# CAMMA-public/SelfPose3d

Measured on AMD Instinct MI355X. Metric: multi-view samples/sec (5-view Panoptic, 80x80x20 voxel), higher is better.
Workload: dtype f32

## Files before the change

include/sp3d.h:

```cpp
#ifndef SP3D_H
#define SP3D_H

#include <stdint.h>

#ifdef __cplusplus
extern "C" {
#endif

#define SP3D_ABI_VERSION 3
#define SP3D_MAX_VIEWS 16
#define SP3D_MAX_TOPK 32

#define SP3D_CAM_STRIDE 64
#define SP3D_CAM_R 0
#define SP3D_CAM_T 9
#define SP3D_CAM_F 12
#define SP3D_CAM_C 14
#define SP3D_CAM_K 16
#define SP3D_CAM_P 19
#define SP3D_CAM_A 21
#define SP3D_CAM_W0 27
#define SP3D_CAM_H0 28
#define SP3D_CAM_FLIP 29
#define SP3D_CAM_RXY 32
// ... 143 lines not shown
                          int64_t sPk, int64_t sQj, int64_t sQk, int conj_p, int conj_q, void *stream);

int sp3d_wino_input(const float *x, float *V, int B, int X, int Y, int Z, int C, void *stream);
int sp3d_wino_output(const float *M, float *y, const float *shift, const float *residual, int mode, int B, int X, int Y,
                     int Z, int O, void *stream);
int sp3d_wino_fused(const float *x, const float *U, float *y, const float *shift, const float *residual, int mode, int B,
                    int X, int Y, int Z, int C, int O, void *stream);

int sp3d_wino_fused_split(const float *x, const void *U3, float *y, const float *shift, const float *residual, int mode, int B,
                          int X, int Y, int Z, int C, int O, void *stream);

int sp3d_wino_fused_split64(const float *x, const void *U3, float *y, const float *shift, const float *residual, int mode,
                            int B, int X, int Y, int Z, int C, int O, void *stream);

int sp3d_conv3_split(const float *x, const void *W3, float *y, const float *shift, const float *residual, int mode, int B,
                     int X, int Y, int Z, int C, int O, void *stream);

int sp3d_upsample2x_scatter(const float *G, float *out, const float *shift, const float *skip, int64_t batch, int X, int Y,
                            int Z, int O, void *stream);

int sp3d_upsample2x_scatter_head(const float *G, float *head, const float *shift, const float *skip, const float *wout,
                                 const float *bout, int64_t batch, int X, int Y, int Z, int O, int J, void *stream);

#define SP3D_GBN_F32 0
#define SP3D_GBN_F64 1
#define SP3D_GBN_REPLICAS 16
#define SP3D_GBN_PLAIN 0
#define SP3D_GBN_RELU 1
#define SP3D_GBN_ADD_RELU 2
int64_t sp3d_gbn_workspace_bytes(int G, int C);
int sp3d_gbn_forward(const void *x, void *y, int dtype, const int32_t *group_of, const int32_t *group_samples, int N,
                     int64_t S, int C, int G, int G_update, const void *weight, const void *bias, void *running_mean,
                     void *running_var, double eps, double momentum, int mode, const void *residual, void *mean,
                     void *invstd, void *scale, void *shift, double *workspace, void *stream);
int sp3d_gbn_backward(const void *x, const void *dy, void *dx, int dtype, const int32_t *group_of,
                      const int32_t *group_samples, int N, int64_t S, int C, int G, const void *weight, const void *mean,
                      const void *invstd, const void *scale, const void *shift, int mode, const void *y,
                      void *grad_residual, void *grad_weight, void *grad_bias, void *k123, double *workspace, void *stream);

#ifdef __cplusplus
}
#endif
#endif
```

selfpose3d_amd/_lib.py:

```python
from __future__ import annotations

import ctypes as C
import os
from typing import Optional, Sequence

import torch

_HERE = os.path.dirname(os.path.abspath(__file__))
_DEFAULT_LIB_PATH = os.path.join(_HERE, "libsp3d.so")
NOPK_LIB_PATH = os.path.join(_HERE, "libsp3d_nopk.so")
LIB_PATH = os.environ.get("SP3D_LIB_PATH") or _DEFAULT_LIB_PATH

LAYOUT_PLANAR = 0
LAYOUT_NHWC = 1
OUT_CHANNELS_LAST = 0x100
HM_BF16 = 0x200
OUT_BF16 = 0x400
HM_ONE_CHANNEL = 0x800
SCATTER_AUTO, SCATTER_PER_TAP, SCATTER_MERGE = 0, 2, 3
MAX_VIEWS = 16
MAX_TOPK = 32
ABI_VERSION = 3

_CTYPES = {"p": C.c_void_p, "i": C.c_int, "l": C.c_int64, "f": C.c_float, "d": C.c_double, "s": C.c_char_p}
# ... 42 lines not shown
    "sp3d_wino_input": "i: pp iiiii p",
    "sp3d_wino_output": "i: pppp iiiiii p",
    "sp3d_wino_fused": "i: ppppp iiiiiii p",
    "sp3d_wino_fused_split": "i: ppppp iiiiiii p",
    "sp3d_wino_fused_split64": "i: ppppp iiiiiii p",
    "sp3d_conv3_split": "i: ppppp iiiiiii p",
    "sp3d_upsample2x_scatter": "i: pppp l iiii p",
    "sp3d_upsample2x_scatter_head": "i: pppppp l iiiii p",
    "sp3d_gbn_workspace_bytes": "l: ii",
    "sp3d_gbn_forward": "i: pp i pp i l iii pppp dd i ppppppp",
    "sp3d_gbn_backward": "i: ppp i pp i l ii ppppp i ppppppp",
}
TUNING_SIGNATURES = {
    "sp3d_unproject_fwd_variant": "i: p i ppppp iiiiiiii p iii p",
    "sp3d_unproject_fwd_plan": "i: iii p iiiiiiiii pppp",
    "sp3d_debug_set_timeline": "i: p",
    "sp3d_debug_stamp": "i: pp",
}
ONE_TRAIN_SIGNATURES = {
    "sp3d_unproject_one_fwd_train": "i: p ii ppppppp iiiiiiii p ii p",
    "sp3d_unproject_one_bwd": "i: ppppp l pp iiiiiiii p ii p",
    "sp3d_unproject_one_bwd_det": "i: ppppp l ppp iiiiiiii p ii p",
}
EXPORTS = list(SIGNATURES)

_lib = None


class Sp3dError(RuntimeError):
    pass


def shared_gpu() -> bool:
    v = os.environ.get("SP3D_SHARED_GPU")
    if v is not None:
        return v.lower() in ("1", "true", "yes", "on")
    if any(os.environ.get(k) not in (None, "") for k in ("HIP_VISIBLE_DEVICES", "CUDA_VISIBLE_DEVICES", "ROCR_VISIBLE_DEVICES",
                                                          "GPU_DEVICE_ORDINAL")):
        return False
    try:
        ranks = int(os.environ.get("LOCAL_WORLD_SIZE", "1"))
        if ranks > 1 and torch.cuda.is_available() and ranks > torch.cuda.device_count():
            import warnings
            warnings.warn(f"selfpose3d_amd: {ranks} local ranks on {torch.cuda.device_count()} GPU(s) - ranks share a GPU: loading "
                          "libsp3d_nopk.so (no packed-fp32 instructions; set SP3D_SHARED_GPU=0 to force the default flavour)")
            return True
    except ValueError:
        pass
    return False


def load():
    global _lib, LIB_PATH
    if _lib is not None:
        return _lib
    if shared_gpu() and LIB_PATH == _DEFAULT_LIB_PATH:
        LIB_PATH = NOPK_LIB_PATH
    if not os.path.exists(LIB_PATH):
        raise Sp3dError(
            f"{LIB_PATH} not found - the HIP extension is not built. Run `python -m selfpose3d_amd.build` "
            "(hipcc, gfx950). There is no CPU fallback for the unprojection path.")
    lib = C.CDLL(LIB_PATH)
    for table, required in ((SIGNATURES, True), (ONE_TRAIN_SIGNATURES, True), (TUNING_SIGNATURES, False)):
        for name, sig in table.items():
            if required or hasattr(lib, name):
                ret, args = sig.split(":")
                fn = getattr(lib, name)
                fn.restype = _CTYPES[ret]
                fn.argtypes = [_CTYPES[a] for a in args.replace(" ", "")]
    if lib.sp3d_abi_version() != ABI_VERSION:
        raise Sp3dError(f"libsp3d.so ABI {lib.sp3d_abi_version()} != binding ABI {ABI_VERSION}; rebuild")
    _lib = lib
    return lib


def check(rc: int, what: str):
    if rc != 0:
        msg = load().sp3d_error_string(rc).decode()
        raise Sp3dError(f"{what} failed: {msg} (code {rc})")


def _stream(device) -> int:
    return torch.cuda.current_stream(device).cuda_stream


def _require_cuda(t: torch.Tensor, name: str):
# ... 645 lines not shown
                               _stream(x.device)), "sp3d_wino_output")
    return y


def wino_fused_conv3d_(x: torch.Tensor, U: torch.Tensor, shift: torch.Tensor, mode: int,
                       residual: Optional[torch.Tensor] = None, U3: Optional[torch.Tensor] = None) -> torch.Tensor:
    lib = load()
    _require_cuda(x, "x")
    B, Cc, X, Y, Z = (int(v) for v in x.shape)
    _require_cl3d_f32(x, "wino_fused_conv3d_")
    O = int(U.shape[2])
    y = _empty_cl3d(B, O, X, Y, Z, x.device)
    if residual is not None:
        residual = _as_cl3d(residual)
    if U3 is None:
        name, weights = "sp3d_wino_fused", U
    else:
        name, weights = ("sp3d_wino_fused_split64" if O == 64 else "sp3d_wino_fused_split"), U3
    check(getattr(lib, name)(x.data_ptr(), weights.data_ptr(), y.data_ptr(), shift.data_ptr(), _opt(residual), int(mode),
                             B, X, Y, Z, Cc, O, _stream(x.device)), name)
    return y


def upsample2x_(x: torch.Tensor, w_gemm: torch.Tensor, shift: torch.Tensor, skip: torch.Tensor) -> torch.Tensor:
    lib = load()
    _require_cuda(x, "x")
    B, Cc, X, Y, Z = (int(v) for v in x.shape)
    _require_cl3d_f32(x, "upsample2x_")
    O = int(w_gemm.shape[1]) // 8
    G = torch.matmul(x.permute(0, 2, 3, 4, 1).reshape(-1, Cc), w_gemm)
    out = _empty_cl3d(B, O, 2 * X, 2 * Y, 2 * Z, x.device)
    skip = _as_cl3d(skip)
    check(lib.sp3d_upsample2x_scatter(G.data_ptr(), out.data_ptr(), shift.data_ptr(), skip.data_ptr(), B, X, Y, Z, O,
                                      _stream(x.device)), "sp3d_upsample2x_scatter")
    return out


def upsample2x_head_(x: torch.Tensor, w_gemm: torch.Tensor, shift: torch.Tensor, skip: torch.Tensor, w_out: torch.Tensor,
                     b_out: torch.Tensor) -> torch.Tensor:
    lib = load()
    _require_cuda(x, "x")
    B, Cc, X, Y, Z = (int(v) for v in x.shape)
    _require_cl3d_f32(x, "upsample2x_head_")
    O = int(w_gemm.shape[1]) // 8
    J = int(w_out.shape[0])
    G = torch.matmul(x.permute(0, 2, 3, 4, 1).reshape(-1, Cc), w_gemm)
    skip = _as_cl3d(skip)
    wo = w_out.reshape(J, O).contiguous().float()
    bo = (b_out if b_out is not None else torch.zeros(J, device=x.device)).contiguous().float()
    head = _empty_cl3d(B, J, 2 * X, 2 * Y, 2 * Z, x.device)
    check(lib.sp3d_upsample2x_scatter_head(G.data_ptr(), head.data_ptr(), shift.data_ptr(), skip.data_ptr(), wo.data_ptr(),
                                           bo.data_ptr(), B, X, Y, Z, O, J, _stream(x.device)), "sp3d_upsample2x_scatter_head")
    return head


class _RenderJoints(torch.autograd.Function):
    @staticmethod
    def forward(ctx, kps, count, h, w, sigma):
        lib = load()
        _require_cuda(kps, "kps")
        N, Pn, J = (int(v) for v in kps.shape[:3])
        k = kps.contiguous().float()
        cnt = None if count is None else count.to(device=kps.device, dtype=torch.int32).contiguous()
        out = torch.empty((N, J, h, w), dtype=torch.float32, device=kps.device)
        check(lib.sp3d_render_joints_fwd(k.data_ptr(), _opt(cnt), N, Pn, J, h, w, float(sigma), out.data_ptr(),
                                         _stream(kps.device)), "sp3d_render_joints_fwd")
        ctx.save_for_backward(k, cnt if cnt is not None else torch.empty(0, device=kps.device))
        ctx.geom = (h, w, float(sigma), cnt is not None, kps.dtype)
        return out if kps.dtype == torch.float32 else out.to(kps.dtype)

    @staticmethod
    def backward(ctx, gout):
        lib = load()
# ... 13 lines not shown
```

selfpose3d_amd/build.py:

```python
from __future__ import annotations

import os
import subprocess
import sys

HERE = os.path.dirname(os.path.abspath(__file__))
CSRC = os.path.join(HERE, "csrc")
SOURCES = ["sp3d_unproject.hip", "sp3d_proposal.hip", "sp3d_epilogue.hip", "sp3d_synth.hip", "sp3d_fftconv.hip", "sp3d_winograd.hip", "sp3d_fft.hip", "sp3d_gbn.hip"]
HEADERS = [os.path.join("..", "pk_src1.py"), "sp3d_device.h", "sp3d_proj_pk.h", "sp3d_tuning.h", "sp3d_twiddles.h", os.path.join("..", "..", "include", "sp3d.h"),
           os.path.join("..", "..", "include", "sp3d_one_train.h")]
LIB = os.path.join(HERE, "libsp3d.so")
HIPCC = os.environ.get("HIPCC", "/opt/rocm/bin/hipcc")
FLAGS = ["--offload-arch=gfx950", "-O3", "-std=c++17", "-ffp-contract=off", "-munsafe-fp-atomics", "-fPIC", "-shared",
         "-Wall", "-Wno-unused-function"]
LINK = ["-L/opt/rocm/lib", "-lhipfft"]


def needs_build() -> bool:
    if not os.path.exists(LIB):
        return True
    t = os.path.getmtime(LIB)
    deps = [os.path.join(CSRC, s) for s in SOURCES + HEADERS] + [os.path.abspath(__file__)]
    return any(os.path.getmtime(d) > t for d in deps if os.path.exists(d))


PER_SOURCE_FLAGS = {"sp3d_winograd.hip": ["-fno-slp-vectorize"],
                    "sp3d_fft.hip": ["-fno-slp-vectorize"], "sp3d_fftconv.hip": ["-fno-slp-vectorize"]}


LLVM_BIN = os.environ.get("SP3D_LLVM_BIN", "/opt/rocm/lib/llvm/bin")

NOPK_LIB = os.path.join(HERE, "libsp3d_nopk.so")
NOPK_FLAGS = ["-DSP3D_NO_PK", "-fno-slp-vectorize", "-Xclang", "-target-feature", "-Xclang", "-packed-fp32-ops"]




def _compile_one(src: str, objdir: str, cflags, verbose: bool, host_flags=()) -> str:
    from . import pk_src1
    base = os.path.join(objdir, src.replace(".hip", ""))
    path = os.path.join(CSRC, src)
    cuid = "-cuid=" + src.replace(".", "_")

    def run(cmd):
        if verbose:
            print(" ".join(cmd))
        subprocess.check_call(cmd)
    if os.environ.get("SP3D_PLAIN_HIPCC", "0") not in ("", "0"):
        flags = cflags + [f for f in NOPK_FLAGS if f not in cflags]
# ... 78 lines not shown
```

selfpose3d_amd/csrc/sp3d_winograd.hip:

```cpp
#include <hip/hip_runtime.h>
#include <stdint.h>

#include "../../include/sp3d.h"

namespace sp3d {

__device__ __forceinline__ void bt4(float &d0, float &d1, float &d2, float &d3)
{
    const float t0 = d0 - d2, t1 = d1 + d2, t2 = d2 - d1, t3 = d1 - d3;
    d0 = t0; d1 = t1; d2 = t2; d3 = t3;
}

__global__ __launch_bounds__(256) void wino_input_kernel(const float *__restrict__ x, float *__restrict__ V, int B, int X,
                                                        int Y, int Z, int C, int TX, int TY, int TZ)
{
    const int64_t T = (int64_t)B * TX * TY * TZ;
    const int64_t gid = (int64_t)blockIdx.x * 256 + threadIdx.x;
    if (gid >= T * C) return;
    const int c = (int)(gid % C);
    int64_t t = gid / C;
    const int tz = (int)(t % TZ); int64_t r = t / TZ;
    const int ty = (int)(r % TY); r /= TY;
    const int tx = (int)(r % TX);
    const int b = (int)(r / TX);
    float d[4][4][4];
#pragma unroll
// ... 119 lines not shown
extern "C" int sp3d_wino_output(const float *M, float *y, const float *shift, const float *residual, int mode, int B, int X,
                                int Y, int Z, int O, void *stream)
{
    if (B <= 0 || X <= 0 || Y <= 0 || Z <= 0 || O <= 0 || mode < 0 || mode > 3) return SP3D_EINVAL;
    if (!M || !y || !shift || (mode >= 2 && !residual)) return SP3D_ENULL;
    const int TX = (X + 1) / 2, TY = (Y + 1) / 2, TZ = (Z + 1) / 2;
    const int64_t n = (int64_t)B * TX * TY * TZ * O;
    if ((n + 255) / 256 > 0x7fffffff) return SP3D_ERANGE;
    const dim3 grid((unsigned)((n + 255) / 256)), block(256);
    hipStream_t s = (hipStream_t)stream;
#define SP3D_WO(MODE_) hipLaunchKernelGGL((wino_output_kernel<MODE_>), grid, block, 0, s, M, y, shift, residual, B, X, Y, Z, O, TX, TY, TZ)
    switch (mode) { case 0: SP3D_WO(0); break; case 1: SP3D_WO(1); break; case 2: SP3D_WO(2); break; default: SP3D_WO(3); }
#undef SP3D_WO
    const hipError_t e = hipGetLastError();
    return e == hipSuccess ? SP3D_OK : (int)e;
}

#ifndef SP3D_W16_ABLATE
#define SP3D_W16_ABLATE 0
#endif

namespace sp3d {

typedef float f32x16 __attribute__((ext_vector_type(16)));
#ifdef SP3D_WF_TIMELINE
__device__ unsigned long long *g_wf_tl = nullptr;
#define WF_STAMP(slot) do { __builtin_amdgcn_sched_barrier(0); if (tl && lane == 0) tl[slot] = __builtin_readcyclecounter(); __builtin_amdgcn_sched_barrier(0); } while (0)
#else
#define WF_STAMP(slot) do { } while (0)
#endif

constexpr int WF_RX = 10, WF_RY = 10, WF_RZ = 6;
constexpr int WF_VS = 8;
constexpr int WF_ROW = WF_RX * WF_VS + 4;
constexpr int WF_LDS = WF_RY * WF_RZ * WF_ROW;

__device__ constexpr int wf_ta(int r) { return r == 0 ? 0 : (r == 1 ? 1 : (r == 2 ? 2 : 1)); }
__device__ constexpr int wf_tb(int r) { return r == 0 ? 2 : (r == 1 ? 2 : (r == 2 ? 1 : 3)); }
__device__ constexpr float wf_sb(int r) { return r == 1 ? 1.0f : -1.0f; }
__device__ constexpr float wf_at(int a, int r) { return a == 0 ? (r < 3 ? 1.0f : 0.0f) : (r == 0 ? 0.0f : (r == 1 ? 1.0f : -1.0f)); }

template <int C, int MODE>
__global__ __launch_bounds__(64) void wino_fused_kernel(const float *__restrict__ x, const float *__restrict__ U,
                                                       float *__restrict__ y, const float *__restrict__ shift,
                                                       const float *__restrict__ res, int B, int X, int Y, int Z, int NBX,
                                                       int NBY, int NBZ)
{
// ... 130 lines not shown
                const int rx = row & 3, ry = (row >> 2) & 3, rz = row >> 4;
                const int xo = min(ox0 + 2 * rx + (a >> 2), X - 1), yo = min(oy0 + 2 * ry + ((a >> 1) & 1), Y - 1);
                const int zo = min(oz0 + 2 * rz + (a & 1), Z - 1);
                rv[v] = res[((((int64_t)b * X + xo) * Y + yo) * Z + zo) * O + t];
            }
        }
#pragma unroll
        for (int v = 0; v < 16; ++v) {
            const int row = 8 * (v >> 2) + (v & 3) + 4 * h;
            const int rx = row & 3, ry = (row >> 2) & 3, rz = row >> 4;
            const int xo = ox0 + 2 * rx + (a >> 2), yo = oy0 + 2 * ry + ((a >> 1) & 1), zo = oz0 + 2 * rz + (a & 1);
            if (xo < X && yo < Y && zo < Z) {
                const int64_t idx = ((((int64_t)b * X + xo) * Y + yo) * Z + zo) * O + t;
                float val = acc[a][v] + sh;
                if (MODE == 2) val += rv[v];
                if (MODE >= 1) val = fmaxf(val, 0.0f);
                if (MODE == 3) val += rv[v];
                y[idx] = val;
            }
        }
    }
}


typedef unsigned u32x4 __attribute__((ext_vector_type(4)));
typedef unsigned u32x2 __attribute__((ext_vector_type(2)));
typedef unsigned u32x4_a8 __attribute__((ext_vector_type(4), aligned(8)));
typedef unsigned u32x2_a8 __attribute__((ext_vector_type(2), aligned(8)));
typedef __bf16 bf16x8 __attribute__((ext_vector_type(8)));
typedef __bf16 bf16x2 __attribute__((ext_vector_type(2)));
typedef float f32x2 __attribute__((ext_vector_type(2)));

__device__ __forceinline__ unsigned pack_bf16(float a, float b)
{
    f32x2 f = {a, b};
    return __builtin_bit_cast(unsigned, __builtin_convertvector(f, bf16x2));
}
__device__ __forceinline__ float bf16_lo(unsigned u) { return __uint_as_float(u << 16); }
__device__ __forceinline__ float bf16_hi(unsigned u) { return __uint_as_float(u & 0xffff0000u); }
__device__ __forceinline__ f32x16 mfma_bf16(u32x4 a, u32x4 b, f32x16 c)
{
    return __builtin_amdgcn_mfma_f32_32x32x16_bf16(__builtin_bit_cast(bf16x8, a), __builtin_bit_cast(bf16x8, b), c, 0, 0, 0);
}

struct WfB { u32x4 mh; u32x2 l; };

template <int C, int MODE>
__global__ __launch_bounds__(64) __attribute__((amdgpu_waves_per_eu(2, 2))) void wino_fused3_kernel(const float *__restrict__ x, const unsigned *__restrict__ U3,
                                                        float *__restrict__ y, const float *__restrict__ shift,
                                                        const float *__restrict__ res, int B, int X, int Y, int Z, int NBX,
                                                        int NBY, int NBZ)
{
    constexpr int O = 32, NCH = C / 8;
    __shared__ __attribute__((aligned(16))) float region[WF_LDS];
    const int lane = threadIdx.x, t = lane & 31, h = lane >> 5;
    int bid = blockIdx.x;
    const int bz = bid % NBZ; bid /= NBZ;
    const int by = bid % NBY; bid /= NBY;
    const int bx = bid % NBX;
    const int b = bid / NBX;
    const int ttx = t & 3, tty = (t >> 2) & 3, ttz = t >> 4;
    const int ox0 = bx * 8, oy0 = by * 8, oz0 = bz * 4;
    const float *rb = region + ((2 * ttz) * WF_RY + 2 * tty) * WF_ROW + (2 * ttx) * WF_VS + 4 * h;

    f32x16 acc[8];
#pragma unroll
// ... 471 lines not shown
constexpr int CD_BX = 16, CD_BY = 8, CD_BZ = 4;
constexpr int CD_RX = CD_BX + 2, CD_RY = CD_BY + 2, CD_RZ = CD_BZ + 2, CD_VOX = 8, CD_ROW = CD_RX * CD_VOX, CD_ZP = CD_RY * CD_ROW + 4;
constexpr int CD_PLANE = CD_RZ * CD_ZP;
constexpr int CD_BUF = 2 * CD_PLANE;
constexpr int CD_NV4 = CD_RX * CD_RY * CD_RZ * 2;
constexpr int CD_PROD = 4;
constexpr int CD_PER = (CD_NV4 + 64 * CD_PROD - 1) / (64 * CD_PROD);
constexpr int CD_BUFS = ((CD_BUF / 4 + 63) / 64) * 256;
#ifndef SP3D_WG_ABLATE
#define SP3D_WG_ABLATE 0
#endif
struct CdRec { u32x4 hl, hh, mm; };


#ifdef SP3D_CD_TIMELINE
__device__ unsigned long long *g_cd_tl = nullptr;
#define CD_STAMP(slot) do { __builtin_amdgcn_sched_barrier(0); if (g_cd_tl && blockIdx.x == 0 && lane == 0 && item < 64) { g_cd_tl[(wave * 64 + item) * 4 + (slot)] = __builtin_readcyclecounter(); \
     \
    if (wave == 0 && (slot) == 0 && item == 0) { g_cd_tl[(7 * 64 + 62) * 4 + 0] = wall_clock64(); g_cd_tl[(7 * 64 + 62) * 4 + 1] = __builtin_readcyclecounter(); } \
    if (wave == 0 && (slot) == 3) { g_cd_tl[(7 * 64 + 63) * 4 + 0] = wall_clock64(); g_cd_tl[(7 * 64 + 63) * 4 + 1] = __builtin_readcyclecounter(); } } __builtin_amdgcn_sched_barrier(0); } while (0)
#else
#define CD_STAMP(slot) do { (void)item; } while (0)
#endif

__device__ __forceinline__ void split3(const float4 a, u32x4 &q0, u32x4 &q1)
{
    const unsigned hi01 = pack_bf16(a.x, a.y), hi23 = pack_bf16(a.z, a.w);
    const float r0 = __builtin_amdgcn_fmed3f(a.x - bf16_lo(hi01), 0.0f, a.x - bf16_lo(hi01));
    const float r1 = __builtin_amdgcn_fmed3f(a.y - bf16_hi(hi01), 0.0f, a.y - bf16_hi(hi01));
    const float r2 = __builtin_amdgcn_fmed3f(a.z - bf16_lo(hi23), 0.0f, a.z - bf16_lo(hi23));
    const float r3 = __builtin_amdgcn_fmed3f(a.w - bf16_hi(hi23), 0.0f, a.w - bf16_hi(hi23));
    const unsigned mid01 = pack_bf16(r0, r1), mid23 = pack_bf16(r2, r3);
    const unsigned lo01 = pack_bf16(r0 - bf16_lo(mid01), r1 - bf16_hi(mid01));
    const unsigned lo23 = pack_bf16(r2 - bf16_lo(mid23), r3 - bf16_hi(mid23));
    q0 = u32x4{lo01, lo23, hi01, hi23};
    q1 = u32x4{hi01, hi23, mid01, mid23};
}

template <int C, int MODE>
__global__ __launch_bounds__(64 * (4 + CD_PROD)) __attribute__((amdgpu_waves_per_eu(2, 2)))
void conv3_split_kernel(const float *__restrict__ x, const unsigned *__restrict__ W3, float *__restrict__ y,
                        const float *__restrict__ shift, const float *__restrict__ res, int B, int X, int Y, int Z, int NBX,
                        int NBY, int NBZ, int nblocks)
{
    constexpr int O = 32, NCH = C / 8;
    extern __shared__ __attribute__((aligned(16))) unsigned cd_lds[];
    const int tid = threadIdx.x, lane = tid & 63, wave = tid >> 6, t = lane & 31, h = lane >> 5;
    const int my_blocks = ((int)blockIdx.x < nblocks) ? (nblocks - 1 - (int)blockIdx.x) / (int)gridDim.x + 1 : 0;
    const int n_items = my_blocks * NCH;
    auto decode = [&](int item, int &b, int &ox0, int &oy0, int &oz0) {
        int bid = (int)blockIdx.x + (item / NCH) * (int)gridDim.x;
        const int bz = bid % NBZ; bid /= NBZ;
        const int by = bid % NBY; bid /= NBY;
        const int bx = bid % NBX;
        b = bid / NBX;
        ox0 = bx * CD_BX; oy0 = by * CD_BY; oz0 = bz * CD_BZ;
    };

    if (wave >= 4) {
        const int pt = tid - 256;
// ... 322 lines not shown
```

selfpose3d_amd/v2v_net.py:

```python
from __future__ import annotations

from typing import NamedTuple, Optional

import torch
import torch.nn as nn
import torch.nn.functional as F


def _bn(c):
    from .grouped_bn import GroupedBatchNorm3d
    return GroupedBatchNorm3d(c)


def _grouped(bn, training: bool) -> bool:
    return training and getattr(bn, "groups", None) is not None


def fft_len(n: int) -> int:
    m = n + (n & 1)
    while True:
        r, odd = m, 0
        for q in (2, 3, 5, 7, 11, 13):
            if q > 2 and r % q == 0:
                odd += 1
# ... 179 lines not shown
        self.spec, self.X, self.Y, self.Z, self.SZ = spec, int(X), int(Y), int(Z), int(SZ)
        self.shape = (int(spec.shape[0]), int(spec.shape[1]), self.X, self.Y, self.Z)
        self.device, self.is_cuda, self.dtype = spec.device, spec.is_cuda, torch.float32


class _Conv(NamedTuple):
    w: torch.Tensor
    shift: torch.Tensor
    u: Optional[torch.Tensor] = None
    split: Optional[torch.Tensor] = None
    direct: Optional[torch.Tensor] = None


class _Res(NamedTuple):
    c1: _Conv
    c2: _Conv
    skip: Optional[torch.Tensor]


class _Up(NamedTuple):
    wT: torch.Tensor
    shift: torch.Tensor
    wg: torch.Tensor


class _FoldedV2V:

    def __init__(self, net: "V2VNet"):
        self.net = net
        self.key = None
        self.layers = {}
        self.spectra = {}
        self.xpad = {}

    def graph_tensors(self):
        return dict(self.layers), dict(self.spectra), dict(self.xpad)

    @staticmethod
    def _key(net):
        ps = list(net.parameters()) + list(net.buffers())
        w3 = net.front_layers[1].res_branch[0].weight
        return (tuple((p.data_ptr(), p._version) for p in ps), str(w3.device), bool(is_cl(w3)))

    def _ensure_built(self):
        key = self._key(self.net)
        if key != self.key:
# ... 2 lines not shown

    @staticmethod
    def _fold(conv, bn, transposed=False):
        s = bn.weight / torch.sqrt(bn.running_var + bn.eps)
        shape = (1, -1, 1, 1, 1) if transposed else (-1, 1, 1, 1, 1)
        w = conv.weight * s.view(shape)
        fmt = torch.channels_last_3d if is_cl(conv.weight) else torch.contiguous_format
        b = conv.bias if conv.bias is not None else torch.zeros_like(bn.running_mean)
        return w.contiguous(memory_format=fmt), ((b - bn.running_mean) * s + bn.bias).contiguous()

    @staticmethod
    def _conv3_record(w, shift):
        from . import _lib
        cout, cin = int(w.shape[0]), int(w.shape[1])
        routes = {conv3_route(cin, cout, (b, 2, 2, 2), True, ws, dc) for b in (1, 1 << 20) for ws in (True, False) for dc in (True, False)}
        if not w.is_cuda or routes == {"library"}:
            return _Conv(w, shift)
        u = _lib.wino_weights(w)
        split = _lib.wino_weights_split(u, 16 if cout == 64 else 8) if "wino_fused_conv3d_" in routes else None
        direct = _lib.conv_weights_split(w) if "conv3_split_" in routes else None
        return _Conv(w, shift, u, split, direct)

    def _build(self):
        n, layers = self.net, {}
        layers["front"] = _Conv(*self._fold(n.front_layers[0].block[0], n.front_layers[0].block[1]))
        ed = n.encoder_decoder
        for name in ("front_res", "encoder_res1", "encoder_res2", "mid_res", "decoder_res2", "decoder_res1", "skip_res1",
                     "skip_res2"):
            blk = n.front_layers[1] if name == "front_res" else getattr(ed, name)
            w1, s1 = self._fold(blk.res_branch[0], blk.res_branch[1])
            w2, s2 = self._fold(blk.res_branch[3], blk.res_branch[4])
            ws = None
            if len(blk.skip_con) > 0:
                ws, ss = self._fold(blk.skip_con[0], blk.skip_con[1])
                s2 = (s2 + ss).contiguous()
            layers[name] = _Res(self._conv3_record(w1, s1), self._conv3_record(w2, s2), ws)
        for name in ("decoder_upsample2", "decoder_upsample1"):
            blk = getattr(ed, name).block
            wT, sT = self._fold(blk[0], blk[1], transposed=True)
            wg = wT.permute(0, 2, 3, 4, 1).reshape(wT.shape[0], 8 * wT.shape[1]).contiguous()
            layers[name] = _Up(wT, sT, wg)
        self.layers, self.spectra, self.xpad = layers, {}, {}

    def _conv3(self, x, c: "_Conv", mode, residual=None):
        from . import _lib
        n, route = self.net, "library"
        split = getattr(n, "wino_split", True)
        if c.u is not None and is_cl(x):
            route = conv3_route(int(c.w.shape[1]), int(c.w.shape[0]), (x.shape[0],) + tuple(x.shape[2:]), n.winograd, split,
                                getattr(n, "direct_conv", True))
        if route == "conv3_split_":
            return _lib.conv3_split_(x, c.direct, c.shift, mode, residual)
        if route == "wino_fused_conv3d_":
            return _lib.wino_fused_conv3d_(x, c.u, c.shift, mode, residual, c.split if split else None)
        if route == "wino_conv3d_":
            return _lib.wino_conv3d_(x, c.u, c.shift, mode, residual)
        return _lib.channel_shift_act_(F.conv3d(x, c.w, None, 1, 1), c.shift, mode, residual)

    def _res(self, x, name):
        r = self.layers[name]
        h = self._conv3(x, r.c1, 1)
        return self._conv3(h, r.c2, 2, x if r.skip is None else self._conv1(x, r.skip))

    _tuned_shapes: "set[tuple]" = set()
# ... 153 lines not shown
        else:
            buf = self._fft_buffer(B, cin, S, x.device)
            buf[:, :, :X, :Y, :Z].copy_(x[:, :cin])
        Yf = _lib.freq_contract(_lib.rfft3d(buf), self._weights_f(w0, S))
        y = _lib.irfft3d_(Yf, S[2])
        cl = is_cl(self.layers["front_res"].c1.w)
        if cl and y.is_contiguous() and y.shape[1] % 4 == 0 and Z % 4 == 0 and 4 * Z * (y.shape[1] + 4) * 4 <= 65536:
            return _lib.crop_shift_act_cl(y, X, Y, Z, s0, True)
        y = y[:, :, :X, :Y, :Z]
        y = y.contiguous(memory_format=torch.channels_last_3d if cl else torch.contiguous_format)
        return _lib.channel_shift_act_(y, s0, 1)

    def _tail(self, x):
        from . import _lib
        x = self._res(x, "front_res")
        skip1 = self._res(x, "skip_res1")
        x = self._res(self._pool(x), "encoder_res1")
        skip2 = self._res(x, "skip_res2")
        x = self._res(self._pool(x), "encoder_res2")
        x = self._res(self._res(x, "mid_res"), "decoder_res2")
        x = self._up2x(x, "decoder_upsample2", skip2)
        x = self._res(x, "decoder_res1")
        o = self.net.output_layer
        wT, sT, wg = self.layers["decoder_upsample1"]
        if self.net.winograd and is_cl(x) and wg.is_cuda and wT.shape[1] == 32 and x.dtype == torch.float32:
            return _lib.upsample2x_head_(x, wg, sT, skip1, o.weight, o.bias)
        x = self._up2x(x, "decoder_upsample1", skip1)
        return self._conv1(x, o.weight, o.bias)

    def _pool(self, x):
        from . import _lib
        if is_cl(x) and x.is_cuda and x.dtype == torch.float32 and x.shape[1] % 4 == 0 and \
                all(int(v) % 2 == 0 for v in x.shape[2:]):
            return _lib.maxpool2x(x)
        return F.max_pool3d(x, 2, 2)

    def _up2x(self, x, name, skip):
        from . import _lib
        wT, sT, wg = self.layers[name]
        if self.net.winograd and is_cl(x) and wg.is_cuda and wT.shape[1] % 4 == 0:
            return _lib.upsample2x_(x, wg, sT, skip)
        return _lib.channel_shift_act_(F.conv_transpose3d(x, wT, None, 2), sT, 3, skip)

    def _conv1(self, x, w, bias=None):
        if self.net.winograd and is_cl(x) and x.is_cuda:
            B, C, X, Y, Z = x.shape
            O = w.shape[0]
            x2 = x.permute(0, 2, 3, 4, 1).reshape(-1, C)
            y = torch.matmul(x2, w.reshape(O, C).t()) if bias is None else torch.addmm(bias, x2, w.reshape(O, C).t())
            return y.view(B, X, Y, Z, O).permute(0, 4, 1, 2, 3)
        return F.conv3d(x, w, bias, 1, 0)


class V2VNet(nn.Module):
    def __init__(self, input_channels: int, output_channels: int):
        super().__init__()
        self.front_layers = nn.Sequential(ConvBnRelu3d(input_channels, 16, 7), Residual3d(16, 32))
        self.encoder_decoder = _EncDec()
        self.output_layer = nn.Conv3d(32, output_channels, 1, 1, 0)
        self.fused_inference = True
        self.fft_front = True
        self.winograd = True
        self.zdft = True
        self.wino_split = True
# ... 83 lines not shown
```

Measured before the change: 2767.

## Fuse transposed-conv GEMM with scatter epilogue and head into one MFMA kernel

Adds a HIP kernel that computes the 2x transposed-conv upsample directly with split-bf16 MFMA (three-piece fp32 emulation), then applies shift, ReLU and skip-add and writes the scattered output in one pass. For the final decoder layer it also applies the 1x1 output head in-kernel through an LDS transpose. This removes the intermediate GEMM result G and its separate scatter kernel, saving a round-trip through global memory. The cost is a more complex kernel restricted to two channel configurations, plus extra MFMA work from the 3-way split.

After: 2825 (median of 6 runs). +2.1%, better.

```diff
diff --git a/include/sp3d.h b/include/sp3d.h
--- a/include/sp3d.h
+++ b/include/sp3d.h
@@ -189,6 +189,8 @@
 int sp3d_upsample2x_scatter_head(const float *G, float *head, const float *shift, const float *skip, const float *wout,
                                  const float *bout, int64_t batch, int X, int Y, int Z, int O, int J, void *stream);
 
+#include "sp3d_upconv.h"
+
 #define SP3D_GBN_F32 0
 #define SP3D_GBN_F64 1
 #define SP3D_GBN_REPLICAS 16
diff --git a/include/sp3d_upconv.h b/include/sp3d_upconv.h
--- /dev/null
+++ b/include/sp3d_upconv.h
@@ -0,0 +1,7 @@
+#ifndef SP3D_UPCONV_H
+#define SP3D_UPCONV_H
+
+int sp3d_upconv2x_fused(const float *x, const void *w_split, const float *shift, const float *skip, const float *w_out,
+                        const float *b_out, float *out, int64_t batch, int X, int Y, int Z, int CIN, int O, int J, void *stream);
+
+#endif
diff --git a/selfpose3d_amd/_lib.py b/selfpose3d_amd/_lib.py
--- a/selfpose3d_amd/_lib.py
+++ b/selfpose3d_amd/_lib.py
@@ -88,6 +88,9 @@
     "sp3d_unproject_one_bwd": "i: ppppp l pp iiiiiiii p ii p",
     "sp3d_unproject_one_bwd_det": "i: ppppp l ppp iiiiiiii p ii p",
 }
+UPCONV_SIGNATURES = {
+    "sp3d_upconv2x_fused": "i: ppppppp l iiiiii p",
+}
 EXPORTS = list(SIGNATURES)
 
 _lib = None
@@ -127,7 +130,8 @@
             f"{LIB_PATH} not found - the HIP extension is not built. Run `python -m selfpose3d_amd.build` "
             "(hipcc, gfx950). There is no CPU fallback for the unprojection path.")
     lib = C.CDLL(LIB_PATH)
-    for table, required in ((SIGNATURES, True), (ONE_TRAIN_SIGNATURES, True), (TUNING_SIGNATURES, False)):
+    for table, required in ((SIGNATURES, True), (ONE_TRAIN_SIGNATURES, True), (UPCONV_SIGNATURES, True),
+                            (TUNING_SIGNATURES, False)):
         for name, sig in table.items():
             if required or hasattr(lib, name):
                 ret, args = sig.split(":")
@@ -819,33 +823,66 @@
     return y
 
 
-def upsample2x_(x: torch.Tensor, w_gemm: torch.Tensor, shift: torch.Tensor, skip: torch.Tensor) -> torch.Tensor:
+def upconv_weights_split(w_gemm: torch.Tensor) -> torch.Tensor:
+    Cc, O = int(w_gemm.shape[0]), int(w_gemm.shape[1]) // 8
+    U = w_gemm.float().reshape(Cc, 8 * O // 32, 32).permute(1, 0, 2).contiguous()
+    pc = wino_weights_split(U, 8)
+    mid, hi, lo = pc[..., 0, :], pc[..., 1, :], pc[..., 2, :]
+    return torch.stack([hi, lo, hi, hi, mid, mid], -2).reshape(8, O // 32, Cc // 8, 2, 32, 6, 4).contiguous()
+
+
+def _require_upconv_split(w_split: torch.Tensor, Cc: int, O: int, x: torch.Tensor):
+    if w_split.device != x.device or w_split.dtype != torch.bfloat16 or not w_split.is_contiguous() or \
+            w_split.numel() != Cc * 8 * O * 6:
+        raise Sp3dError(f"w_split must be upconv_weights_split(w_gemm) of the ({Cc}, {8 * O}) weight on {x.device}; got "
+                        f"{tuple(w_split.shape)}, {w_split.dtype}, {w_split.device}, contiguous={w_split.is_contiguous()}")
+
+
+def upconv_fused_covers(Cc: int, O: int, head: bool) -> bool:
+    if os.environ.get("SP3D_FUSE_UPCONV", "1") in ("0", ""):
+        return False
+    return (Cc, O, bool(head)) in ((64, 32, True), (128, 64, False))
+
+
+def upsample2x_(x: torch.Tensor, w_gemm: torch.Tensor, shift: torch.Tensor, skip: torch.Tensor,
+                w_split: Optional[torch.Tensor] = None) -> torch.Tensor:
     lib = load()
     _require_cuda(x, "x")
     B, Cc, X, Y, Z = (int(v) for v in x.shape)
     _require_cl3d_f32(x, "upsample2x_")
     O = int(w_gemm.shape[1]) // 8
-    G = torch.matmul(x.permute(0, 2, 3, 4, 1).reshape(-1, Cc), w_gemm)
     out = _empty_cl3d(B, O, 2 * X, 2 * Y, 2 * Z, x.device)
     skip = _as_cl3d(skip)
+    if w_split is not None and upconv_fused_covers(Cc, O, False):
+        _require_upconv_split(w_split, Cc, O, x)
+        check(lib.sp3d_upconv2x_fused(x.data_ptr(), w_split.data_ptr(), shift.data_ptr(), skip.data_ptr(), None, None,
+                                      out.data_ptr(), B, X, Y, Z, Cc, O, 0, _stream(x.device)), "sp3d_upconv2x_fused")
+        return out
+    G = torch.matmul(x.permute(0, 2, 3, 4, 1).reshape(-1, Cc), w_gemm)
     check(lib.sp3d_upsample2x_scatter(G.data_ptr(), out.data_ptr(), shift.data_ptr(), skip.data_ptr(), B, X, Y, Z, O,
                                       _stream(x.device)), "sp3d_upsample2x_scatter")
     return out
 
 
 def upsample2x_head_(x: torch.Tensor, w_gemm: torch.Tensor, shift: torch.Tensor, skip: torch.Tensor, w_out: torch.Tensor,
-                     b_out: torch.Tensor) -> torch.Tensor:
+                     b_out: torch.Tensor, w_split: Optional[torch.Tensor] = None) -> torch.Tensor:
     lib = load()
     _require_cuda(x, "x")
     B, Cc, X, Y, Z = (int(v) for v in x.shape)
     _require_cl3d_f32(x, "upsample2x_head_")
     O = int(w_gemm.shape[1]) // 8
     J = int(w_out.shape[0])
-    G = torch.matmul(x.permute(0, 2, 3, 4, 1).reshape(-1, Cc), w_gemm)
     skip = _as_cl3d(skip)
     wo = w_out.reshape(J, O).contiguous().float()
+    head = _empty_cl3d(B, J, 2 * X, 2 * Y, 2 * Z, x.device)
+    if w_split is not None and J <= 32 and upconv_fused_covers(Cc, O, True):
+        _require_upconv_split(w_split, Cc, O, x)
+        bo = None if b_out is None else b_out.contiguous().float()
+        check(lib.sp3d_upconv2x_fused(x.data_ptr(), w_split.data_ptr(), shift.data_ptr(), skip.data_ptr(), wo.data_ptr(),
+                                      _opt(bo), head.data_ptr(), B, X, Y, Z, Cc, O, J, _stream(x.device)), "sp3d_upconv2x_fused")
+        return head
+    G = torch.matmul(x.permute(0, 2, 3, 4, 1).reshape(-1, Cc), w_gemm)
     bo = (b_out if b_out is not None else torch.zeros(J, device=x.device)).contiguous().float()
-    head = _empty_cl3d(B, J, 2 * X, 2 * Y, 2 * Z, x.device)
     check(lib.sp3d_upsample2x_scatter_head(G.data_ptr(), head.data_ptr(), shift.data_ptr(), skip.data_ptr(), wo.data_ptr(),
                                            bo.data_ptr(), B, X, Y, Z, O, J, _stream(x.device)), "sp3d_upsample2x_scatter_head")
     return head
diff --git a/selfpose3d_amd/build.py b/selfpose3d_amd/build.py
--- a/selfpose3d_amd/build.py
+++ b/selfpose3d_amd/build.py
@@ -6,9 +6,9 @@
 
 HERE = os.path.dirname(os.path.abspath(__file__))
 CSRC = os.path.join(HERE, "csrc")
-SOURCES = ["sp3d_unproject.hip", "sp3d_proposal.hip", "sp3d_epilogue.hip", "sp3d_synth.hip", "sp3d_fftconv.hip", "sp3d_winograd.hip", "sp3d_fft.hip", "sp3d_gbn.hip"]
-HEADERS = [os.path.join("..", "pk_src1.py"), "sp3d_device.h", "sp3d_proj_pk.h", "sp3d_tuning.h", "sp3d_twiddles.h", os.path.join("..", "..", "include", "sp3d.h"),
-           os.path.join("..", "..", "include", "sp3d_one_train.h")]
+SOURCES = ["sp3d_unproject.hip", "sp3d_proposal.hip", "sp3d_epilogue.hip", "sp3d_upconv.hip", "sp3d_synth.hip", "sp3d_fftconv.hip", "sp3d_winograd.hip", "sp3d_fft.hip", "sp3d_gbn.hip"]
+HEADERS = [os.path.join("..", "pk_src1.py"), "sp3d_device.h", "sp3d_proj_pk.h", "sp3d_split.h", "sp3d_tuning.h", "sp3d_twiddles.h", os.path.join("..", "..", "include", "sp3d.h"),
+           os.path.join("..", "..", "include", "sp3d_one_train.h"), os.path.join("..", "..", "include", "sp3d_upconv.h")]
 LIB = os.path.join(HERE, "libsp3d.so")
 HIPCC = os.environ.get("HIPCC", "/opt/rocm/bin/hipcc")
 FLAGS = ["--offload-arch=gfx950", "-O3", "-std=c++17", "-ffp-contract=off", "-munsafe-fp-atomics", "-fPIC", "-shared",
@@ -24,7 +24,7 @@
     return any(os.path.getmtime(d) > t for d in deps if os.path.exists(d))
 
 
-PER_SOURCE_FLAGS = {"sp3d_winograd.hip": ["-fno-slp-vectorize"],
+PER_SOURCE_FLAGS = {"sp3d_winograd.hip": ["-fno-slp-vectorize"], "sp3d_upconv.hip": ["-fno-slp-vectorize"],
                     "sp3d_fft.hip": ["-fno-slp-vectorize"], "sp3d_fftconv.hip": ["-fno-slp-vectorize"]}
 
 
diff --git a/selfpose3d_amd/csrc/sp3d_split.h b/selfpose3d_amd/csrc/sp3d_split.h
--- /dev/null
+++ b/selfpose3d_amd/csrc/sp3d_split.h
@@ -0,0 +1,53 @@
+#ifndef SP3D_SPLIT_H
+#define SP3D_SPLIT_H
+#include <hip/hip_runtime.h>
+
+namespace sp3d {
+
+typedef float f32x16 __attribute__((ext_vector_type(16)));
+typedef unsigned u32x4 __attribute__((ext_vector_type(4)));
+typedef unsigned u32x2 __attribute__((ext_vector_type(2)));
+typedef unsigned u32x4_a8 __attribute__((ext_vector_type(4), aligned(8)));
+typedef unsigned u32x2_a8 __attribute__((ext_vector_type(2), aligned(8)));
+typedef __bf16 bf16x8 __attribute__((ext_vector_type(8)));
+typedef __bf16 bf16x2 __attribute__((ext_vector_type(2)));
+typedef float f32x2 __attribute__((ext_vector_type(2)));
+
+__device__ __forceinline__ unsigned pack_bf16(float a, float b)
+{
+    f32x2 f = {a, b};
+    return __builtin_bit_cast(unsigned, __builtin_convertvector(f, bf16x2));
+}
+__device__ __forceinline__ float bf16_lo(unsigned u) { return __uint_as_float(u << 16); }
+__device__ __forceinline__ float bf16_hi(unsigned u) { return __uint_as_float(u & 0xffff0000u); }
+__device__ __forceinline__ f32x16 mfma_bf16(u32x4 a, u32x4 b, f32x16 c)
+{
+    return __builtin_amdgcn_mfma_f32_32x32x16_bf16(__builtin_bit_cast(bf16x8, a), __builtin_bit_cast(bf16x8, b), c, 0, 0, 0);
+}
+
+__device__ __forceinline__ void split3(const float4 a, u32x4 &q0, u32x4 &q1)
+{
+    const unsigned hi01 = pack_bf16(a.x, a.y), hi23 = pack_bf16(a.z, a.w);
+    const float r0 = __builtin_amdgcn_fmed3f(a.x - bf16_lo(hi01), 0.0f, a.x - bf16_lo(hi01));
+    const float r1 = __builtin_amdgcn_fmed3f(a.y - bf16_hi(hi01), 0.0f, a.y - bf16_hi(hi01));
+    const float r2 = __builtin_amdgcn_fmed3f(a.z - bf16_lo(hi23), 0.0f, a.z - bf16_lo(hi23));
+    const float r3 = __builtin_amdgcn_fmed3f(a.w - bf16_hi(hi23), 0.0f, a.w - bf16_hi(hi23));
+    const unsigned mid01 = pack_bf16(r0, r1), mid23 = pack_bf16(r2, r3);
+    const unsigned lo01 = pack_bf16(r0 - bf16_lo(mid01), r1 - bf16_hi(mid01));
+    const unsigned lo23 = pack_bf16(r2 - bf16_lo(mid23), r3 - bf16_hi(mid23));
+    q0 = u32x4{lo01, lo23, hi01, hi23};
+    q1 = u32x4{hi01, hi23, mid01, mid23};
+}
+
+typedef unsigned u32x6 __attribute__((ext_vector_type(6)));
+__device__ __forceinline__ u32x6 split3_pieces(const float4 a)
+{
+    u32x4 q0, q1;
+    split3(a, q0, q1);
+    return u32x6{q0.x, q0.y, q0.z, q0.w, q1.z, q1.w};
+}
+__device__ __forceinline__ u32x4 split3_q0(const u32x6 p) { return __builtin_shufflevector(p, p, 0, 1, 2, 3); }
+__device__ __forceinline__ u32x4 split3_q1(const u32x6 p) { return __builtin_shufflevector(p, p, 2, 3, 4, 5); }
+
+}
+#endif
diff --git a/selfpose3d_amd/csrc/sp3d_upconv.hip b/selfpose3d_amd/csrc/sp3d_upconv.hip
--- /dev/null
+++ b/selfpose3d_amd/csrc/sp3d_upconv.hip
@@ -0,0 +1,200 @@
+#include <hip/hip_runtime.h>
+#include <stdint.h>
+
+#include "../../include/sp3d.h"
+#include "sp3d_split.h"
+
+namespace sp3d {
+
+constexpr int UC_STAGE = 8 * 2 * 32 * 3;
+constexpr int UC_PER = UC_STAGE / 256;
+constexpr int UC_SCR = 33;
+
+template <int CIN, int O, bool HEAD, bool MULTI>
+__global__ __launch_bounds__(256) __attribute__((amdgpu_waves_per_eu(2))) void upconv2x_fused_kernel(
+    const float *__restrict__ x, const u32x4 *__restrict__ W, const float *__restrict__ shift, const float *__restrict__ skip,
+    const float *__restrict__ wout, const float *__restrict__ bout, float *__restrict__ out, int n_in, int X, int Y, int Z, int J,
+    int ny, int taps_per_block)
+{
+    constexpr int KS = CIN / 64, OB = O / 32, SPT = KS * OB;
+    extern __shared__ __attribute__((aligned(16))) u32x4 uc_lds[];
+    const int tid = threadIdx.x, lane = tid & 63, wave = tid >> 6, t = lane & 31, h = lane >> 5;
+    const int tile = (int)blockIdx.x / ny;
+    const int tap0 = ((int)blockIdx.x % ny) * taps_per_block;
+    const int n0 = tile * 128 + wave * 32;
+    const int nvalid = n_in - n0;
+    const int nstages = taps_per_block * SPT;
+
+    float *scr = reinterpret_cast<float *>(uc_lds + 2 * UC_STAGE) + wave * 32 * UC_SCR;
+    float *wo = reinterpret_cast<float *>(uc_lds + 2 * UC_STAGE) + 4 * 32 * UC_SCR;
+    if (HEAD) {
+        for (int i = tid; i < J * 32; i += 256) wo[i] = wout[i];
+        if (tid < 32) wo[32 * 32 + tid] = (bout && tid < J) ? bout[tid] : 0.0f;
+    }
+
+    u32x4 wreg[UC_PER];
+    auto fetch = [&](int q) {
+        const int tap = tap0 + q / SPT, ks = (q % SPT) / OB, ob = q % OB;
+        const u32x4 *p = W + (int64_t)((tap * OB + ob) * KS + ks) * UC_STAGE + tid;
+#pragma unroll
+        for (int r = 0; r < UC_PER; ++r) wreg[r] = p[256 * r];
+    };
+    auto stash = [&](int buf) {
+        u32x4 *p = uc_lds + buf * UC_STAGE + tid;
+#pragma unroll
+        for (int r = 0; r < UC_PER; ++r) p[256 * r] = wreg[r];
+    };
+    fetch(0);
+
+    const int na = min(n0 + t, n_in - 1);
+    const float *xp = x + (int64_t)na * CIN + 4 * h;
+    u32x6 ap[8];
+    auto load_a = [&](int ks) {
+        float4 d[8];
+#pragma unroll
+        for (int kc = 0; kc < 8; ++kc) d[kc] = *reinterpret_cast<const float4 *>(xp + 64 * ks + 8 * kc);
+#pragma unroll
+        for (int kc = 0; kc < 8; ++kc) ap[kc] = split3_pieces(d[kc]);
+    };
+    if (KS == 1) load_a(0);
+    int base;
+    {
+        int n = na;
+        const int z = n % Z; n /= Z;
+        const int y = n % Y; n /= Y;
+        const int xx = n % X;
+        const int b = n / X;
+        base = ((b * 2 * X + 2 * xx) * 2 * Y + 2 * y) * 2 * Z + 2 * z;
+    }
+    unsigned vb[16];
+#pragma unroll
+    for (int v = 0; v < 16; ++v) vb[v] = (unsigned)__shfl(base, 8 * (v >> 2) + (v & 3) + 4 * h) * O + t;
+
+    auto tap_off = [&](int tap) { return (((tap >> 2) * 2 * Y) + ((tap >> 1) & 1)) * 2 * Z + (tap & 1); };
+    float sk[OB][16];
+    auto fetch_skip = [&](int tap, int ob) {
+        const int toff = tap_off(tap);
+#pragma unroll
+        for (int v = 0; v < 16; ++v) sk[ob][v] = skip[vb[v] + (unsigned)(toff * O + ob * 32)];
+    };
+#pragma unroll
+    for (int ob = 0; ob < OB; ++ob) fetch_skip(tap0, ob);
+    stash(0);
+    __syncthreads();
+
+    int buf = 0, q = 0;
+    for (int tap = tap0; tap < tap0 + taps_per_block; ++tap) {
+        const int toff = tap_off(tap);
+        f32x16 acc[OB];
+#pragma unroll
+        for (int ob = 0; ob < OB; ++ob)
+#pragma unroll
+            for (int v = 0; v < 16; ++v) acc[ob][v] = 0.0f;
+#pragma unroll
+        for (int ks = 0; ks < KS; ++ks) {
+            if (KS > 1) load_a(ks);
+#pragma unroll
+            for (int ob = 0; ob < OB; ++ob, ++q) {
+                fetch(min(q + 1, nstages - 1));
+                const u32x4 *wl = uc_lds + buf * UC_STAGE + (h * 32 + t) * 3;
+#pragma unroll
+                for (int kc = 0; kc < 8; ++kc) {
+                    const u32x4 hl = wl[kc * 192], hh = wl[kc * 192 + 1], mm = wl[kc * 192 + 2];
+                    acc[ob] = mfma_bf16(split3_q0(ap[kc]), hl, acc[ob]);
+                    acc[ob] = mfma_bf16(split3_q1(ap[kc]), hh, acc[ob]);
+                    acc[ob] = mfma_bf16(split3_q1(ap[kc]), mm, acc[ob]);
+                }
+                if (ks == KS - 1) {
+                    const float sh = shift[ob * 32 + t];
+                    const unsigned ob_off = (unsigned)(toff * O + ob * 32);
+                    float val[16];
+#pragma unroll
+                    for (int v = 0; v < 16; ++v) {
+                        const float a = acc[ob][v] + sh;
+                        val[v] = (a < 0.0f ? 0.0f : a) + sk[ob][v];
+                    }
+                    if (MULTI) fetch_skip(min(tap + 1, tap0 + taps_per_block - 1), ob);
+                    if (!HEAD) {
+                        if (nvalid >= 32) {
+#pragma unroll
+                            for (int v = 0; v < 16; ++v) out[vb[v] + ob_off] = val[v];
+                        } else {
+#pragma unroll
+                            for (int v = 0; v < 16; ++v)
+                                if (8 * (v >> 2) + (v & 3) + 4 * h < nvalid) out[vb[v] + ob_off] = val[v];
+                        }
+                    } else {
+#pragma unroll
+                        for (int v = 0; v < 16; ++v) scr[(8 * (v >> 2) + (v & 3) + 4 * h) * UC_SCR + t] = val[v];
+                        __builtin_amdgcn_fence(__ATOMIC_RELEASE, "wavefront");
+                        __builtin_amdgcn_wave_barrier();
+                        float c[16];
+#pragma unroll
+                        for (int i = 0; i < 16; ++i) c[i] = scr[t * UC_SCR + 16 * h + i];
+                        __builtin_amdgcn_fence(__ATOMIC_RELEASE, "wavefront");
+                        __builtin_amdgcn_wave_barrier();
+                        float *hp = out + (unsigned)(base + toff) * (unsigned)J;
+                        const bool mine = h == 0 && t < nvalid;
+                        for (int j = 0; j < J; ++j) {
+                            const float *wj = wo + j * 32 + 16 * h;
+                            float p = 0.0f;
+#pragma unroll
+                            for (int i4 = 0; i4 < 4; ++i4) {
+                                const float4 w4 = *reinterpret_cast<const float4 *>(wj + 4 * i4);
+                                p = fmaf(c[4 * i4 + 3], w4.w, fmaf(c[4 * i4 + 2], w4.z, fmaf(c[4 * i4 + 1], w4.y, fmaf(c[4 * i4], w4.x, p))));
+                            }
+                            p += __shfl_xor(p, 32);
+                            if (mine) hp[j] = p + wo[32 * 32 + j];
+                        }
+                    }
+                }
+                stash(buf ^ 1);
+                __syncthreads();
+                buf ^= 1;
+            }
+        }
+    }
+}
+
+}
+
+extern "C" int sp3d_upconv2x_fused(const float *x, const void *w_split, const float *shift, const float *skip,
+                                   const float *w_out, const float *b_out, float *out, int64_t batch, int X, int Y, int Z,
+                                   int CIN, int O, int J, void *stream)
+{
+    using namespace sp3d;
+    const bool head = w_out != nullptr;
+    if (batch <= 0 || X <= 0 || Y <= 0 || Z <= 0 || CIN <= 0 || O <= 0 || (head && (J <= 0 || J > 32))) return SP3D_EINVAL;
+    if (!x || !w_split || !shift || !skip || !out) return SP3D_ENULL;
+    if (!((CIN == 64 && O == 32 && head) || (CIN == 128 && O == 64 && !head))) return SP3D_EUNSUPPORTED;
+    if ((reinterpret_cast<uintptr_t>(x) | reinterpret_cast<uintptr_t>(w_split)) & 15) return SP3D_EUNSUPPORTED;
+    const int64_t n_in = batch * X * Y * Z;
+    if (n_in * 8 * (head && J > O ? J : O) > 0x7fffffff) return SP3D_ERANGE;
+    const int tiles = (int)((n_in + 127) / 128);
+    int ny = 1;
+    while (ny < 8 && (int64_t)tiles * ny < 480) ny *= 2;
+    const dim3 grid((unsigned)(tiles * ny)), block(256);
+    const size_t lds = (size_t)2 * UC_STAGE * 16 + (head ? (size_t)(4 * 32 * UC_SCR + 32 * 32 + 32) * sizeof(float) : 0);
+    hipStream_t s = (hipStream_t)stream;
+    const u32x4 *w = reinterpret_cast<const u32x4 *>(w_split);
+    if (head) {
+        int dev = 0;
+        { const hipError_t ed = hipGetDevice(&dev); if (ed != hipSuccess) return (int)ed; }
+        if (dev < 0 || dev >= 64) dev = 63;
+        const bool multi = ny < 8;
+        const auto kern = multi ? upconv2x_fused_kernel<64, 32, true, true> : upconv2x_fused_kernel<64, 32, true, false>;
+        static bool attr_dev[2][64] = {};
+        if (!attr_dev[multi][dev] || dev == 63) {
+            const hipError_t ea = hipFuncSetAttribute(reinterpret_cast<const void *>(kern),
+                                                      hipFuncAttributeMaxDynamicSharedMemorySize, (int)lds);
+            if (ea != hipSuccess) return (int)ea;
+            attr_dev[multi][dev] = true;
+        }
+        hipLaunchKernelGGL(kern, grid, block, lds, s, x, w, shift, skip, w_out, b_out, out, (int)n_in, X, Y, Z, J, ny, 8 / ny);
+    } else {
+        const auto kern = ny < 8 ? upconv2x_fused_kernel<128, 64, false, true> : upconv2x_fused_kernel<128, 64, false, false>;
+        hipLaunchKernelGGL(kern, grid, block, lds, s, x, w, shift, skip, w_out, b_out, out, (int)n_in, X, Y, Z, 0, ny, 8 / ny);
+    }
+    const hipError_t e = hipGetLastError();
+    return e == hipSuccess ? SP3D_OK : (int)e;
+}
diff --git a/selfpose3d_amd/csrc/sp3d_winograd.hip b/selfpose3d_amd/csrc/sp3d_winograd.hip
--- a/selfpose3d_amd/csrc/sp3d_winograd.hip
+++ b/selfpose3d_amd/csrc/sp3d_winograd.hip
@@ -2,6 +2,7 @@
 #include <stdint.h>
 
 #include "../../include/sp3d.h"
+#include "sp3d_split.h"
 
 namespace sp3d {
 
@@ -167,7 +168,6 @@
 
 namespace sp3d {
 
-typedef float f32x16 __attribute__((ext_vector_type(16)));
 #ifdef SP3D_WF_TIMELINE
 __device__ unsigned long long *g_wf_tl = nullptr;
 #define WF_STAMP(slot) do { __builtin_amdgcn_sched_barrier(0); if (tl && lane == 0) tl[slot] = __builtin_readcyclecounter(); __builtin_amdgcn_sched_barrier(0); } while (0)
@@ -344,26 +344,6 @@
     }
 }
 
-
-typedef unsigned u32x4 __attribute__((ext_vector_type(4)));
-typedef unsigned u32x2 __attribute__((ext_vector_type(2)));
-typedef unsigned u32x4_a8 __attribute__((ext_vector_type(4), aligned(8)));
-typedef unsigned u32x2_a8 __attribute__((ext_vector_type(2), aligned(8)));
-typedef __bf16 bf16x8 __attribute__((ext_vector_type(8)));
-typedef __bf16 bf16x2 __attribute__((ext_vector_type(2)));
-typedef float f32x2 __attribute__((ext_vector_type(2)));
-
-__device__ __forceinline__ unsigned pack_bf16(float a, float b)
-{
-    f32x2 f = {a, b};
-    return __builtin_bit_cast(unsigned, __builtin_convertvector(f, bf16x2));
-}
-__device__ __forceinline__ float bf16_lo(unsigned u) { return __uint_as_float(u << 16); }
-__device__ __forceinline__ float bf16_hi(unsigned u) { return __uint_as_float(u & 0xffff0000u); }
-__device__ __forceinline__ f32x16 mfma_bf16(u32x4 a, u32x4 b, f32x16 c)
-{
-    return __builtin_amdgcn_mfma_f32_32x32x16_bf16(__builtin_bit_cast(bf16x8, a), __builtin_bit_cast(bf16x8, b), c, 0, 0, 0);
-}
 
 struct WfB { u32x4 mh; u32x2 l; };
 
@@ -881,20 +861,6 @@
 #else
 #define CD_STAMP(slot) do { (void)item; } while (0)
 #endif
-
-__device__ __forceinline__ void split3(const float4 a, u32x4 &q0, u32x4 &q1)
-{
-    const unsigned hi01 = pack_bf16(a.x, a.y), hi23 = pack_bf16(a.z, a.w);
-    const float r0 = __builtin_amdgcn_fmed3f(a.x - bf16_lo(hi01), 0.0f, a.x - bf16_lo(hi01));
-    const float r1 = __builtin_amdgcn_fmed3f(a.y - bf16_hi(hi01), 0.0f, a.y - bf16_hi(hi01));
-    const float r2 = __builtin_amdgcn_fmed3f(a.z - bf16_lo(hi23), 0.0f, a.z - bf16_lo(hi23));
-    const float r3 = __builtin_amdgcn_fmed3f(a.w - bf16_hi(hi23), 0.0f, a.w - bf16_hi(hi23));
-    const unsigned mid01 = pack_bf16(r0, r1), mid23 = pack_bf16(r2, r3);
-    const unsigned lo01 = pack_bf16(r0 - bf16_lo(mid01), r1 - bf16_hi(mid01));
-    const unsigned lo23 = pack_bf16(r2 - bf16_lo(mid23), r3 - bf16_hi(mid23));
-    q0 = u32x4{lo01, lo23, hi01, hi23};
-    q1 = u32x4{hi01, hi23, mid01, mid23};
-}
 
 template <int C, int MODE>
 __global__ __launch_bounds__(64 * (4 + CD_PROD)) __attribute__((amdgpu_waves_per_eu(2, 2)))
diff --git a/selfpose3d_amd/v2v_net.py b/selfpose3d_amd/v2v_net.py
--- a/selfpose3d_amd/v2v_net.py
+++ b/selfpose3d_amd/v2v_net.py
@@ -225,6 +225,7 @@
     wT: torch.Tensor
     shift: torch.Tensor
     wg: torch.Tensor
+    split: Optional[torch.Tensor] = None
 
 
 class _FoldedV2V:
@@ -273,6 +274,7 @@
         return _Conv(w, shift, u, split, direct)
 
     def _build(self):
+        from . import _lib
         n, layers = self.net, {}
         layers["front"] = _Conv(*self._fold(n.front_layers[0].block[0], n.front_layers[0].block[1]))
         ed = n.encoder_decoder
@@ -290,7 +292,8 @@
             blk = getattr(ed, name).block
             wT, sT = self._fold(blk[0], blk[1], transposed=True)
             wg = wT.permute(0, 2, 3, 4, 1).reshape(wT.shape[0], 8 * wT.shape[1]).contiguous()
-            layers[name] = _Up(wT, sT, wg)
+            fused = wg.is_cuda and (int(wT.shape[0]), int(wT.shape[1])) in ((128, 64), (64, 32))
+            layers[name] = _Up(wT, sT, wg, _lib.upconv_weights_split(wg) if fused else None)
         self.layers, self.spectra, self.xpad = layers, {}, {}
 
     def _conv3(self, x, c: "_Conv", mode, residual=None):
@@ -490,9 +493,9 @@
         x = self._up2x(x, "decoder_upsample2", skip2)
         x = self._res(x, "decoder_res1")
         o = self.net.output_layer
-        wT, sT, wg = self.layers["decoder_upsample1"]
+        wT, sT, wg, w3 = self.layers["decoder_upsample1"]
         if self.net.winograd and is_cl(x) and wg.is_cuda and wT.shape[1] == 32 and x.dtype == torch.float32:
-            return _lib.upsample2x_head_(x, wg, sT, skip1, o.weight, o.bias)
+            return _lib.upsample2x_head_(x, wg, sT, skip1, o.weight, o.bias, w3)
         x = self._up2x(x, "decoder_upsample1", skip1)
         return self._conv1(x, o.weight, o.bias)
 
@@ -505,9 +508,9 @@
 
     def _up2x(self, x, name, skip):
         from . import _lib
-        wT, sT, wg = self.layers[name]
+        wT, sT, wg, w3 = self.layers[name]
         if self.net.winograd and is_cl(x) and wg.is_cuda and wT.shape[1] % 4 == 0:
-            return _lib.upsample2x_(x, wg, sT, skip)
+            return _lib.upsample2x_(x, wg, sT, skip, w3)
         return _lib.channel_shift_act_(F.conv_transpose3d(x, wT, None, 2), sT, 3, skip)
 
     def _conv1(self, x, w, bias=None):
```
